# thanhndv212/figaroh-plus

Measured on AMD Instinct MI355X. Metric: samples/sec regressor build + TSQR solve, UR10 6-DoF, higher is better.
Workload: dtype f64

## Files before the change

figaroh_plus_amd/_lib.py:

```python
from __future__ import annotations

import ctypes as C
import os

import numpy as np

_HERE = os.path.dirname(os.path.abspath(__file__))
LIB_PATH = os.environ.get("FIGH_LIB_PATH") or os.path.join(_HERE, "libfigh.so")

ABI_VERSION = 116

FIGH_OK = 0
ERR_INVALID, ERR_NO_DEVICE, ERR_ALLOC, ERR_UNSUPPORTED, ERR_COMM = -1, -2, -3, -4, -5

MODE_JOINT_TORQUE, MODE_EXT_WRENCH = 0, 1
FLAG_FRICTION, FLAG_ACT_INERTIA, FLAG_OFFSET, FLAG_TX40, FLAG_GENERIC, FLAG_BLOCKED_INPUTS = 1, 2, 4, 8, 256, 512
FLAG_COMPACT_BLOCKS = 2048
FLAG_FORCE_COMPACT = 8192
FLAG_LINK_COMPACT = 4096
FLAG_ZEROS_PRESENT = 1024

_c_double_p = C.POINTER(C.c_double)
_c_int32_p = C.POINTER(C.c_int32)

SIGNATURES = {
# ... 48 lines not shown
    "figh_regressor_link_layout": (C.c_int, [C.c_void_p, C.c_int, C.c_int, C.c_int, _c_int32_p, C.POINTER(C.c_int)]),
    "figh_tsqr_selected_blocks": (C.c_int, [C.c_void_p, C.c_int64, C.c_int64, C.c_void_p, C.c_int, C.c_double, C.c_int,
                                            C.c_int, C.c_int, C.c_void_p, C.c_void_p, C.c_void_p, C.c_void_p, C.c_void_p,
                                            C.c_void_p, C.c_double, C.c_void_p, C.c_void_p, C.c_void_p]),
    "figh_block_rows_residuals": (C.c_int, [C.c_void_p, C.c_int, _c_int32_p, C.c_int, C.c_void_p, C.c_void_p]),
    "figh_tsqr_selected": (C.c_int, [C.c_void_p, C.c_int64, C.c_int64, C.c_void_p, C.c_int, C.c_double, C.c_int, C.c_int,
                                     C.c_int, C.c_void_p, C.c_double, C.c_void_p, C.c_void_p]),
    "figh_regressor_tsqr_fused": (C.c_int, [C.c_void_p, C.c_int, C.c_int64, C.c_void_p, C.c_void_p, C.c_void_p, C.c_void_p,
                                            C.c_int64, C.c_void_p, C.c_void_p, C.c_int, C.c_void_p, C.c_double,
                                            C.c_void_p]),
    "figh_chain_host_tail": (C.c_int, [C.c_void_p]),
    "figh_chain_pass_fused": (C.c_int, [C.c_void_p, C.c_int, C.c_int64, C.c_void_p, C.c_void_p, C.c_void_p, C.c_void_p,
                                        C.c_int64, C.c_void_p, C.c_int, C.c_void_p, C.c_double, C.c_double, C.c_void_p,
                                        C.c_void_p, C.c_size_t, C.c_void_p, C.POINTER(C.c_int), C.c_void_p]),
    "figh_tsqr_merge_base": (C.c_int, [C.c_void_p, C.c_int, C.c_int, C.c_int, C.c_double, C.c_void_p]),
    "figh_compact_rows": (C.c_int, [C.c_void_p, C.c_int64, C.c_int, C.c_int64, C.c_void_p, C.c_int, C.c_double, C.c_void_p,
                                    C.c_int64, C.c_void_p, C.POINTER(C.c_int64)]),
    "figh_base_permutation": (C.c_int, [C.c_void_p, C.c_int, C.c_int, C.c_double, C.c_void_p]),
    "figh_regressor_colsq": (C.c_int, [C.c_void_p, C.c_int, C.c_int, C.c_int, C.c_int64, C.c_void_p, C.c_void_p,
                                       C.c_void_p, C.c_int64, C.c_void_p]),
    "figh_regressor_tsqr": (C.c_int, [C.c_void_p, C.c_int, C.c_int, C.c_int, C.c_int64, C.c_void_p, C.c_void_p,
                                      C.c_void_p, C.c_void_p, C.c_int, C.c_void_p, _c_double_p, C.c_int, C.c_int64,
                                      C.c_void_p]),
    "figh_regressor_tsqr_norms": (C.c_int, [C.c_void_p, C.c_int, C.c_int, C.c_int, C.c_int64, C.c_void_p, C.c_void_p,
                                            C.c_void_p, C.c_void_p, C.c_int, C.c_void_p, _c_double_p, C.c_int, C.c_int64,
                                            C.c_void_p, C.c_void_p]),
    "figh_regressor_tsqr_batch": (C.c_int, [C.c_void_p, C.c_int, C.c_int, C.c_int, C.c_int64, C.c_int64, C.c_void_p,
                                            C.c_void_p, C.c_void_p, C.c_void_p, C.c_int, C.c_void_p, C.c_void_p]),
    "figh_regressor_tsqr_batch_fused": (C.c_int, [C.c_void_p, C.c_int, C.c_int64, C.c_int64, C.c_void_p, C.c_void_p,
                                                  C.c_void_p, C.c_void_p, C.c_int, C.c_void_p, C.c_void_p]),
# ... 652 lines not shown
                     kept_mask_u8, tail):
    changed = C.c_int(0)
    rc = load().figh_chain_pass_fused(model.handle, flags, N, d_q.ptr, d_v.ptr, d_a.ptr, d_W.ptr, ldw, d_kept.ptr, n,
                                      d_tau.ptr if d_tau is not None else None, tol_qr, tol_e, d_pack.ptr, h_pack, pack_bytes,
                                      kept_mask_u8.ctypes.data, C.byref(changed), tail.ref)
    if rc == ERR_UNSUPPORTED:
        return None
    check(rc)
    return not changed.value


def tsqr_merge_base(d_Rs, count, nc, n_free, tol_qr, d_Rk):
    check(load().figh_tsqr_merge_base(d_Rs.ptr, count, nc, n_free, tol_qr, d_Rk.ptr))


def repack_samples(d_src, N, width):
    d_dst = DeviceArray((((N + 63) // 64) * 64 * width,), np.float64)
    check(load().figh_repack_samples(d_src.ptr, N, width, d_dst.ptr))
    return d_dst
```

figaroh_plus_amd/csrc/figh_fused.hip:

```cpp
#include <algorithm>
#include <cmath>
#include <cstdlib>
#include <string>
#include <type_traits>

#include "figh_internal.h"
#include "figh_spatial.h"
#include "figh_chain.h"
#include "figh_wave.h"
#include "figh_tsqr_narrow.h"

namespace figh {

typedef double f64x2 __attribute__((ext_vector_type(2)));

struct FusedCtrl {
    int produced;
    int taken;
    int claimed;
    int pad[5];
};

__device__ __forceinline__ int lds_peek(const int *p) {
    return __hip_atomic_load(p, __ATOMIC_RELAXED, __HIP_MEMORY_SCOPE_WORKGROUP);
// ... 415 lines not shown
    if (!attr_set) {
        FIGH_HIP(hipFuncSetAttribute(reinterpret_cast<const void *>(&fused_chain_tsqr_kernel<NJ, TRAJ>),
                                     hipFuncAttributeMaxDynamicSharedMemorySize, 160 * 1024));
        attr_set = true;
    }
    plan->P = chain_params<NJ>(m);
    plan->tri = (int)tri;
    plan->ncons = ncons;
    plan->lds = sizeof(double) * (fixed + (size_t)ncons * tri);
    return FIGH_OK;
}

template <int NJ>
static int launch_fused(const figh_model_s *m, int flags, long N, const double *q, const double *v, const double *a,
                        double *W, const double *tau, const int *d_kept, int n, double *d_colsq, double **Rws_out,
                        long *count_out) {
    using G = FusedGeom<NJ>;
    const int nc = n + (tau ? 1 : 0);
    FusedPlan<NJ> pl;
    if (int rc = fused_plan<NJ, false>(m, nc, &pl)) return rc;
    const int cus = cu_count(), ncons = pl.ncons;
    const long ntiles_s = (N + 63) / 64;
    long grid = cus < ntiles_s / 2 ? cus : ntiles_s / 2;
    double *part = static_cast<double *>(workspace(sizeof(double) * grid * G::NPROD * G::NC, kWsRegressorNorms));
    double *Rws = static_cast<double *>(workspace(sizeof(double) * (size_t)nc * nc * (grid * ncons + 1), kWsLevel0TriOrWrench));
    if (!part || !Rws) return FIGH_ERR_ALLOC;
    {
        ProfileScope scope("fused_chain_tsqr", true);
        FIGH_LAUNCH_TIMED((fused_chain_tsqr_kernel<NJ, false>), dim3((unsigned)grid), dim3(64 * (G::NPROD + ncons)), pl.lds,
                          pl.P, flags, N, q, v, a, W, tau, d_kept, n, nc, part, Rws, ncons, pl.tri, null_pivot_sq());
    }
    launch_reduce_partials(part, (int)(grid * G::NPROD), G::NC, d_colsq);
    FIGH_HIP(hipGetLastError());
    *Rws_out = Rws;
    *count_out = grid * ncons;
    return FIGH_OK;
}

static long fused_batch_slices(long B, long n_per, int cus) {
    const long tiles = (n_per + 63) / 64;
    return std::max(1L, std::min(tiles, (long)cus / B));
}

template <int NJ>
static int launch_fused_batch(const figh_model_s *m, int flags, long B, long n_per, const double *q, const double *v,
                              const double *a, const int *d_cols, int n, const double *d_R_stack, double *d_R_out) {
    using G = FusedGeom<NJ>;
// ... 26 lines not shown
        FIGH_HIP(hipGetLastError());
        if (nb == 1) return FIGH_OK;
        cur = dst;
        cnt = nb;
        extra = nullptr;
        slot = slot == kWsMergeA ? kWsMergeB : kWsMergeA;
    }
}

}

using namespace figh;

static int fused_pass_launch(figh_model_t model, int flags, int64_t N, const double *d_q, const double *d_v, const double *d_a,
                             double *d_W, int64_t ldw, double *d_colsq, const int32_t *d_kept, int n, const double *d_tau,
                             double **Rws, long *count) {
    FIGH_REQUIRE(N >= 0 && n >= 1, "bad shape");
    const DevModel &h = model->host;
    const int nc = n + (d_tau ? 1 : 0);
    const int ncols = 14 * h.nlinks;
    if (!model->is_chain || (flags & (FIGH_FLAG_TX40 | FIGH_FLAG_GENERIC | FIGH_FLAG_BLOCKED_INPUTS)) || ldw != ncols ||
        (reinterpret_cast<uintptr_t>(d_W) % 16) != 0 || nc > 64 || n > ncols || N < 4096) {
        set_error("fused regressor + TSQR: serial chain, joint-torque mode, packed 16-byte aligned W, at most 64 columns "
                  "(tau included) and at least 4096 samples");
        return FIGH_ERR_UNSUPPORTED;
    }
    if (int rc = ensure_device()) return rc;
    const int f = flags & 7;
    switch (h.nlinks) {
        case 5:
            return launch_fused<5>(model, f, (long)N, d_q, d_v, d_a, d_W, d_tau, d_kept, n, d_colsq, Rws, count);
        case 6:
            return launch_fused<6>(model, f, (long)N, d_q, d_v, d_a, d_W, d_tau, d_kept, n, d_colsq, Rws, count);
        case 7:
            return launch_fused<7>(model, f, (long)N, d_q, d_v, d_a, d_W, d_tau, d_kept, n, d_colsq, Rws, count);
        default:
            set_error("fused regressor + TSQR: serial chains of 5 to 7 joints (LDS: two tile buffers + three consumer triangles)");
            return FIGH_ERR_UNSUPPORTED;
    }
}

extern "C" int figh_regressor_tsqr_fused(figh_model_t model, int flags, int64_t N, const double *d_q, const double *d_v,
                                         const double *d_a, double *d_W, int64_t ldw, double *d_colsq,
                                         const int32_t *d_kept, int n, const double *d_tau, double tol_qr,
                                         double *d_R_out) {
    FIGH_REQUIRE(model && d_q && d_v && d_a && d_W && d_colsq && d_kept && d_R_out, "NULL pointer");
    double *Rws = nullptr;
    long count = 0;
    if (int rc = fused_pass_launch(model, flags, N, d_q, d_v, d_a, d_W, ldw, d_colsq, d_kept, n, d_tau, &Rws, &count))
        return rc;
    return tsqr_reduce_stack(Rws, count, n + (d_tau ? 1 : 0), n, tol_qr, d_R_out);
}

extern "C" int figh_chain_pass_fused(figh_model_t model, int flags, int64_t N, const double *d_q, const double *d_v,
                                     const double *d_a, double *d_W, int64_t ldw, const int32_t *d_kept, int n,
                                     const double *d_tau, double tol_qr, double tol_e, double *d_pack, double *h_pack,
                                     size_t pack_bytes, const uint8_t *h_kept_mask, int *changed, figh_host_tail_t *tail) {
    FIGH_REQUIRE(model && d_q && d_v && d_a && d_W && d_kept && d_pack && h_pack && h_kept_mask && changed && tail,
                 "NULL pointer");
    FIGH_REQUIRE(tol_qr >= 0.0, "figh_chain_pass_fused: the rank decision needs tol_qr >= 0");
    const int ncols = 14 * model->host.nlinks, nc = n + (d_tau ? 1 : 0);
    const size_t sel_words = (size_t)(2 + 2 * ncols + 1) / 2;
    const size_t words = (size_t)ncols + sel_words + (size_t)(nc > 0 ? (nc + 1) * nc : 0);
    FIGH_REQUIRE(n >= 1 && pack_bytes >= sizeof(double) * words, "figh_chain_pass_fused: the pack is [colsq | sel | rows]");
    FIGH_REQUIRE(tail->n == n && (tail->with_tau != 0) == (d_tau != nullptr), "figh_chain_pass_fused: tail of another shape");
    double *d_colsq = d_pack, *d_rows = d_pack + ncols + sel_words;
    int32_t *d_sel = reinterpret_cast<int32_t *>(d_pack + ncols);
    double *Rws = nullptr;
    long count = 0;
    if (int rc = fused_pass_launch(model, flags, N, d_q, d_v, d_a, d_W, ldw, d_colsq, d_kept, n, d_tau, &Rws, &count)) return rc;
    if (int rc = tsqr_reduce_stack(Rws, count, nc, n, tol_qr, d_rows)) return rc;
    if (int rc = figh_select_columns(d_colsq, ncols, tol_e, 14, d_sel)) return rc;
    FIGH_HIP(hipMemcpyAsync(h_pack, d_pack, sizeof(double) * words, hipMemcpyDeviceToHost, stream()));
    FIGH_HIP(hipStreamSynchronize(stream()));
    const int32_t *mask_now = reinterpret_cast<const int32_t *>(h_pack + ncols) + 2 + ncols;
    *changed = 0;
    for (int c = 0; c < ncols; ++c)
        if ((mask_now[c] != 0) != (h_kept_mask[c] != 0)) {
            *changed = 1;
            return FIGH_OK;
        }
    tail->rows_k = h_pack + ncols + sel_words;
    return figh_chain_host_tail(tail);
}

static constexpr int64_t kFusedBatchMinSamples = 64;

extern "C" int figh_regressor_tsqr_batch_fused(figh_model_t model, int flags, int64_t B, int64_t n_per, const double *d_q,
// ... 40 lines not shown
```

figaroh_plus_amd/csrc/figh_internal.h:

```cpp
#pragma once

#include <hip/hip_runtime.h>
#include <hip/hip_ext.h>

#include <cstdint>
#include <cstdio>
#include <string>

#include "figh.h"

namespace figh {

constexpr int kMaxJoints = 64;

struct DevModel {
    int njoints, nq, nv, nlinks;
    int parents[kMaxJoints];
    int jtype[kMaxJoints];
    int idx_q[kMaxJoints];
    int idx_v[kMaxJoints];
    int body_mask[kMaxJoints];
    int depth[kMaxJoints];
    double axis[kMaxJoints][3];
    double placement[kMaxJoints][12];
// ... 172 lines not shown
    int njobs = 0, ncfull = 0, nfull = 0;
};
int launch_tsqr_group(std::vector<Tsqr2Job> &jobs, int ncfull, int nfull, int cus, GroupEmbed *later = nullptr);
int launch_tsqr_group_embed(const GroupEmbed &e);
int tsqr_reduce_stack(const double *d_Rs, long count, int nc, int n_free, double tol_qr, double *d_out);
int launch_tsqr_wide_pairs(const double *stack, long count, int nc, double *Rws_out);
int launch_tsqr_wide_single(const double *W, long rows, long ldw, const int *col_idx, int n, int nc, double *R_out);
int launch_tsqr_wide_batch(const double *W, long ldw, const int *col_idx, int n, int nc, long B, long n_per, int rps,
                           long seg_stride, long wgs, double *Rws_out);
int tsqr_wide_tile_rows(int nc);
int launch_tsqr_wide_chain(const double *W, long rows, long ldw, const int *col_idx, int n, const double *tau,
                           const double *d_blkw, long rows_per_blk, int nc, long nwg, double *Rws_out);

int launch_tsqr_tree(const double *Rs, long count, int nc, int n_free, double tol, double *d_out, double *d_rows_out);

int launch_tsqr_stream(const double *Rs, long count, int nc, int n_free, double tol, double *d_out, double *d_rows_out);

#define FIGH_HIP(expr)                                                                          \
    do {                                                                                        \
        hipError_t _e = (expr);                                                                 \
        if (_e != hipSuccess) {                                                                 \
            figh::set_error(std::string(#expr) + ": " + hipGetErrorString(_e));                 \
            return FIGH_ERR_NO_DEVICE;                                                          \
        }                                                                                       \
    } while (0)

#define FIGH_REQUIRE(cond, msg)              \
    do {                                     \
        if (!(cond)) {                       \
            figh::set_error(msg);            \
            return FIGH_ERR_INVALID;         \
// ... 5 lines not shown
```

figaroh_plus_amd/csrc/figh_linalg.hip:

```cpp
#include <cstdlib>
#include <algorithm>
#include <cstdio>
#include <type_traits>
#include <vector>

#include "figh_internal.h"
#include "figh_wave.h"
#include "figh_tsqr_narrow.h"
#include "figh_tsqr_narrow_kernel.h"

namespace figh {


template <int NCC, int NRC, bool LDSRED, bool RLAST = false>
__global__ __launch_bounds__(64, (NCC <= 4 || RLAST) ? 2 : 1) void tsqr2_kernel(
    const double *__restrict__ W, const long rows, const long ldw, const int *__restrict__ col_idx, const int n,
    const double *__restrict__ tau, const double *__restrict__ blkw, const long rows_per_blk,
    double *__restrict__ Rws, const int nc, const int *__restrict__ tile_first, const double null2) {
    tsqr2_level0_body<NCC, NRC, LDSRED, RLAST>(W, rows, ldw, col_idx, n, tau, blkw, rows_per_blk, Rws, nc, tile_first,
                                        (long)blockIdx.x, (long)gridDim.x, null2);
}



// ... 16 lines not shown
            s0 += x0 * x0;
            s1 += x1 * x1;
        }
        if (r < re) {
            const double x0 = W[r * ldw + c];
            s0 += x0 * x0;
        }
        part[(long)blockIdx.x * cols + c] = s0 + s1;
    }
}

__global__ __launch_bounds__(256) void reduce_partials_kernel(const double *__restrict__ part, int nblocks, int ncols,
                                                              double *__restrict__ out) {
    __shared__ double sm[256];
    const int c = blockIdx.x;
    double s = 0.0;
    for (int b = threadIdx.x; b < nblocks; b += 256) s += part[(long)b * ncols + c];
    sm[threadIdx.x] = s;
    __syncthreads();
    for (int w = 128; w > 0; w >>= 1) {
        if ((int)threadIdx.x < w) sm[threadIdx.x] += sm[threadIdx.x + w];
        __syncthreads();
    }
    if (threadIdx.x == 0) out[c] = sm[0];
}

void launch_reduce_partials(const double *part, int nblocks, int ncols, double *out) {
    hipLaunchKernelGGL(reduce_partials_kernel, dim3(ncols), dim3(256), 0, stream(), part, nblocks, ncols, out);
}

__global__ __launch_bounds__(256) void gather_cols_kernel(const double *__restrict__ W, long rows, long ldw,
                                                          const int *__restrict__ col_idx, int n,
                                                          double *__restrict__ out, long ldo) {
    const long total = rows * n;
    for (long e = (long)blockIdx.x * blockDim.x + threadIdx.x; e < total; e += (long)gridDim.x * blockDim.x) {
        const long r = e / n;
        const int c = (int)(e - r * n);
        out[r * ldo + c] = W[r * ldw + col_idx[c]];
// ... 83 lines not shown
            const int lim = 14 * b < ncols ? 14 * b : ncols;
            int f = 0;
            for (int c = 0; c < lim; ++c) f += kept[c];
            first[b] = f;
        }
        __syncthreads();
        const long t = (long)blockIdx.x * 256 + tid;
        if (t < ntiles) {
            const long r0 = t * 64, r1 = (r0 + 63 < rows ? r0 + 63 : rows - 1);
            int f = first[r0 / rows_per_block];
            for (long b = r0 / rows_per_block + 1; b <= r1 / rows_per_block; ++b) f = min(f, first[b]);
            tile_first[t] = f;
        }
    }
    if (blockIdx.x != 0) return;
    int total = 0;
    for (int c = 0; c < ncols; ++c) total += kept[c];
    for (int c = tid; c < ncols; c += 256) {
        int pos = 0;
        for (int e = 0; e < c; ++e) pos += kept[e];
        if (kept[c]) sel[2 + pos] = (link_pos ? max(link_pos[c / 14], 0) : c / 14) * link_stride + c % 14;
        if (c >= total) sel[2 + c] = 0;
        sel[2 + ncols + c] = kept[c];
    }
    if (tid == 0) {
        sel[0] = total;
        sel[1] = ncols;
    }
}

__global__ __launch_bounds__(256) void split_force_columns_kernel(const int *__restrict__ kept, const int n,
                                                                  const int link_stride, int *__restrict__ fsel,
                                                                  const int force_compact) {
    __shared__ int flag[1024];
    const int tid = threadIdx.x;
    for (int c = tid; c < n; c += 256) flag[c] = (kept[c] % link_stride) >= 6;
    __syncthreads();
    for (int c = tid; c < n; c += 256) {
        if (!flag[c]) continue;
        int pos = 0;
        for (int e = 0; e < c; ++e) pos += flag[e];
        const int p = kept[c] / link_stride, s = kept[c] % link_stride;
        fsel[pos] = force_compact ? 16 * (p >> 2) + 4 * (p & 3) + (s - 6) : kept[c];
// ... 496 lines not shown
int figh::tsqr_reduce_stack(const double *d_Rs, long count, int nc, int n_free, double tol_qr, double *d_out) {
    if (tol_qr < 0.0) return figh_tsqr_merge(d_Rs, (int)count, nc, d_out);
    double *one = static_cast<double *>(workspace(sizeof(double) * (size_t)nc * nc, kWsOneTri));
    if (!one) return FIGH_ERR_ALLOC;
    if (count == 1) {
        if (nc <= 80) return reveal_triangle(d_Rs, nc, n_free, tol_qr, d_out);
        FIGH_HIP(hipMemcpyAsync(one, d_Rs, sizeof(double) * (size_t)nc * nc, hipMemcpyDeviceToDevice, stream()));
        return reveal_triangle(one, nc, n_free, tol_qr, d_out);
    }
    if (nc <= 80) {
        const int rc = merge_one_launch(d_Rs, count, nc, n_free, tol_qr, one, d_out);
        if (rc != FIGH_ERR_UNSUPPORTED) return rc;
    }
    if (int rc = tsqr_reduce(d_Rs, count, nc, one)) return rc;
    return reveal_triangle(one, nc, n_free, tol_qr, d_out);
}

static int tsqr_selected_impl(const double *d_W, int64_t rows, int64_t ldw, const double *d_colsq, int ncols, double tol_e,
                              int link_stride, int nblocks, int n_expected, const double *d_tau, double tol_qr, int32_t *d_sel,
                              double *d_R_out, const int32_t *d_link_pos) {
    FIGH_REQUIRE(d_W && d_colsq && d_sel, "NULL device pointer");
    if (int rc = check_selected(ncols, link_stride, rows > 0 && n_expected <= ncols,
                                nblocks >= 0 && nblocks <= kMaxJoints && (nblocks == 0 || rows % nblocks == 0),
                                "rows must be a multiple of the hint blocks"))
        return rc;
    const int nc = n_expected + (d_tau ? 1 : 0);
    const bool hinted = nblocks > 0 && n_expected > 0 && nc <= 80 && rows / nblocks >= 1;
    const long ntiles = (rows + 63) / 64;
    int *d_tile = nullptr;
    if (hinted) {
// ... 299 lines not shown
    if (int rc = ensure_device()) return rc;
    ProfileScope scope("block_rows_residuals");
    hipLaunchKernelGGL(block_rows_residuals_kernel, dim3((unsigned)nblocks), dim3(256), 0, stream(), d_rows, bo, nc, d_v, d_r2);
    FIGH_HIP(hipGetLastError());
    return FIGH_OK;
}

int figh_tsqr_merge_base(const double *d_Rs, int count, int nc, int n_free, double tol_qr, double *d_Rk_out) {
    FIGH_REQUIRE(d_Rs && d_Rk_out, "NULL device pointer");
    FIGH_REQUIRE(count >= 1 && nc >= 1 && nc <= 512 && n_free >= 1 && n_free <= nc, "bad shape");
    FIGH_REQUIRE(tol_qr >= 0.0, "tol_qr must be non-negative");
    if (int rc = ensure_device()) return rc;
    return tsqr_reduce_stack(d_Rs, count, nc, n_free, tol_qr, d_Rk_out);
}

}
```

figaroh_plus_amd/csrc/figh_tsqr_stream.hip:

```cpp
#include "figh_internal.h"
#include "figh_wave.h"

namespace figh {

constexpr unsigned long long kPoison = 0xFFFBADC0FFEE5EEDull;
constexpr int kDepth = 1;

struct StreamPlan {
    int nlevels;
    int nb[6];
    int first[6];
    int nin[6];
};

__device__ __forceinline__ double ld_coherent(const double *p) {
    return __longlong_as_double(__hip_atomic_load(reinterpret_cast<const long long *>(p), __ATOMIC_RELAXED,
                                                  __HIP_MEMORY_SCOPE_AGENT));
}
__device__ __forceinline__ void st_coherent(double *p, const double v) {
    __hip_atomic_store(reinterpret_cast<long long *>(p), __double_as_longlong(v), __ATOMIC_RELAXED,
                       __HIP_MEMORY_SCOPE_AGENT);
}
__device__ __forceinline__ bool is_poison(const double v) { return (unsigned long long)__double_as_longlong(v) == kPoison; }

// ... 245 lines not shown
        if (c.lane_g == 0 && 16 * (P + cc) + c.lane_c >= c.pad) Rrow[16 * (P + cc) + c.lane_c] = 0.0 - wj;
    }
}

template <int P, int NCC>
__device__ __forceinline__ void solo_stream_panels(double (&T)[solo_tile_n(NCC)], double (&S)[kDepth][NCC], const SoloCtx &c) {
#define FIGH_RSTEP(KK) \
    if (16 * P + KK >= c.pad) solo_stream_step<KK, P, NCC>(T, S, c);
    FIGH_RSTEP(0) FIGH_RSTEP(1) FIGH_RSTEP(2) FIGH_RSTEP(3) FIGH_RSTEP(4) FIGH_RSTEP(5) FIGH_RSTEP(6) FIGH_RSTEP(7)
    FIGH_RSTEP(8) FIGH_RSTEP(9) FIGH_RSTEP(10) FIGH_RSTEP(11) FIGH_RSTEP(12) FIGH_RSTEP(13) FIGH_RSTEP(14)
    FIGH_RSTEP(15)
#undef FIGH_RSTEP
    if constexpr (P + 1 < NCC) solo_stream_panels<P + 1, NCC>(T, S, c);
}

template <int NCC, int FANR, int NW>
__global__ __launch_bounds__(64 * NW) void tsqr_stream_kernel(const double *in, double *sbuf, double *out, double *rows_out,
                                                              const StreamPlan plan, const int nc, const int n_free,
                                                              const double tol) {
    static_assert(NW == 8, "positions are dealt to eight waves");
    constexpr int FAN = 4 * FANR;
    __shared__ double pw[2][NW][16 * NCC];
    const int lane = threadIdx.x & 63, wave = __builtin_amdgcn_readfirstlane(threadIdx.x >> 6);
    const int lane_c = lane & 15, lane_g = lane >> 4;
    const int pad = 16 * NCC - nc;
    const int b = blockIdx.x;
    const long tri = (long)nc * nc;
    if (b < plan.first[plan.nlevels]) {
        int l = 0;
        while (l + 1 < plan.nlevels && b >= plan.first[l + 1]) ++l;
        const int bl = b - plan.first[l];
        const bool root = l == plan.nlevels - 1;
        MergeCtx<NCC, FANR> c;
        c.nc = nc;
        c.pad = pad;
        c.wave = wave;
        c.lane_c = lane_c;
// ... 15 lines not shown
            c.coff[r] = (c.have[r] ? ch : 0) * (int)tri + lane_c - pad;
        }
        c.stream = (!root || rows_out) ? sbuf + (long)b * tri : nullptr;
        c.plain = (root && out) ? out : nullptr;
        if (c.plain) {
            for (int e = threadIdx.x; e < nc * nc; e += 64 * NW) c.plain[e] = 0.0;
        }
        double T[merge_tile_n(NCC, FANR)];
#pragma unroll
        for (int e = 0; e < merge_tile_n(NCC, FANR); ++e) T[e] = 0.0;
        __syncthreads();
        stream_panels<0, NCC, FANR, NW>(T, c, pw);
        return;
    }
    for (int e = threadIdx.x; e < nc * nc; e += 64 * NW) rows_out[e] = 0.0;
    __syncthreads();
    if (wave != 0) return;
    SoloCtx c;
    c.nc = nc;
    c.pad = pad;
    c.lane_c = lane_c;
    c.lane_g = lane_g;
    c.n_free = n_free;
    c.tol = tol;
    c.rows_out = rows_out;
    if (plan.nlevels == 0) {
        c.R = in;
        c.repoison = nullptr;
    } else {
        double *rb = sbuf + (long)(plan.first[plan.nlevels] - 1) * tri;
// ... 5 lines not shown
    for (int e = 0; e < solo_tile_n(NCC); ++e) T[e] = 0.0;
#pragma unroll
    for (int dd = 0; dd < kDepth; ++dd)
#pragma unroll
        for (int e = 0; e < NCC; ++e) S[dd][e] = 0.0;
    solo_stream_panels<0, NCC>(T, S, c);
}

__global__ __launch_bounds__(256) void poison_fill_kernel(double *p, const long n) {
    for (long e = (long)blockIdx.x * 256 + threadIdx.x; e < n; e += (long)gridDim.x * 256)
        p[e] = __longlong_as_double((long long)kPoison);
}

template <int NCC, int FANR>
static int launch_stream(const double *Rs, long count, int nc, int n_free, double tol, double *d_out, double *d_rows_out,
                         int cus) {
    constexpr int FAN = 4 * FANR;
    StreamPlan plan{};
    int l = 0, total = 0;
    long cnt = count;
    while (cnt > 0) {
        if (l >= 5) return FIGH_ERR_UNSUPPORTED;
        const long nb = (cnt + FAN - 1) / FAN;
        plan.nin[l] = (int)cnt;
        plan.nb[l] = (int)nb;
        plan.first[l] = total;
        total += (int)nb;
        ++l;
        if (nb == 1) break;
        cnt = nb;
    }
    plan.nlevels = l;
    plan.first[l] = total;
    const int grid = total + (d_rows_out ? 1 : 0);
    if (grid > cus || grid < 1 || count * nc * nc >= (1L << 31)) return FIGH_ERR_UNSUPPORTED;
    static double *sbuf = nullptr;
    static long sbuf_elems = 0;
    const long need = (long)(total > 0 ? total : 1) * nc * nc;
    if (need > sbuf_elems) {
        if (sbuf) {
            FIGH_HIP(hipStreamSynchronize(stream()));
            FIGH_HIP(hipFree(sbuf));
            sbuf = nullptr;
            sbuf_elems = 0;
        }
        const long want = need + need / 4 + 4096;
        FIGH_HIP(hipMalloc(&sbuf, sizeof(double) * want));
        sbuf_elems = want;
        hipLaunchKernelGGL(poison_fill_kernel, dim3(256), dim3(256), 0, stream(), sbuf, want);
        FIGH_HIP(hipGetLastError());
    }
    static int occ = -1;
    if (occ < 0) {
        int v = 0;
        if (hipOccupancyMaxActiveBlocksPerMultiprocessor(&v, tsqr_stream_kernel<NCC, FANR, 8>, 512, 0) != hipSuccess) v = 0;
        occ = v;
    }
    if (occ < 1) return FIGH_ERR_UNSUPPORTED;
    hipLaunchKernelGGL((tsqr_stream_kernel<NCC, FANR, 8>), dim3((unsigned)grid), dim3(512), 0, stream(), Rs, sbuf, d_out,
                       d_rows_out, plan, nc, n_free, tol);
    FIGH_HIP(hipGetLastError());
    return FIGH_OK;
}

int launch_tsqr_stream(const double *Rs, long count, int nc, int n_free, double tol, double *d_out, double *d_rows_out) {
    int dev = 0, cus = 256;
    (void)hipGetDevice(&dev);
    if (hipDeviceGetAttribute(&cus, hipDeviceAttributeMultiprocessorCount, dev) != hipSuccess || cus <= 0) cus = 256;
    ProfileScope scope("tsqr_tree");
    if (nc <= 64) return launch_stream<4, 4>(Rs, count, nc, n_free, tol, d_out, d_rows_out, cus);
    if (nc <= 80) return launch_stream<5, 2>(Rs, count, nc, n_free, tol, d_out, d_rows_out, cus);
    return FIGH_ERR_UNSUPPORTED;
}

}
```

figaroh_plus_amd/pipeline.py:

```python
import numpy as np

from . import _lib
from .device import GpuMatrix
from .tools import qrdecomposition as qrd
from .tools.regressor import build_regressor_device


class Exchange:

    world_size = 1
    rank = 0

    @property
    def collective(self):
        return self.world_size > 1

    def sum_columns(self, d_colsq, ncols):
        return d_colsq.to_host()

    def sum_columns_device(self, d_colsq, ncols):
        if self.world_size > 1:
            total = np.ascontiguousarray(self.sum_columns(d_colsq, ncols), dtype=np.float64)
            _lib.check(_lib.load().figh_memcpy_h2d(d_colsq.ptr, total.ctypes.data, total.nbytes))

# ... 520 lines not shown
        pin = self._landing()
        total_rows = W.rows * ex.world_size
        tail = self._tail_args(n, with_tau, total_rows)
        ok = _lib.chain_pass_fused(handle, flags, self.N, self.d_q, self.d_v, self.d_a, W.buf, W.ld, d_kept, n, self.d_tau,
                                   self.tol_qr, self.tol_e, self._d_pack, pin.array.ctypes.data, 8 * pin.size,
                                   mask.view(np.uint8), tail)
        if ok is None:
            self.fuse = False
            return None
        if not ok:
            self._fused_kept = None
            return None
        self.fused_passes += 1
        self._n_expected = n
        idx_e, params_r = self._kept_lists(mask)
        out = self._native_out(tail, n, params_r, idx_e, pin.array[:ncols].copy(), with_tau, total_rows, strings)
        with _single_threaded_blas(n):
            pass
        return out

    def _tail_args(self, n, with_tau, total_rows):
        tail = self._host_tail
        if tail is None or tail.n != n or tail.with_tau != bool(with_tau):
            tail = self._host_tail = _lib.HostTail(n, with_tau)
        s = tail.s
        s.tol_qr, s.total_rows, s.pieces = self.tol_qr, int(total_rows), self._level0_pieces(total_rows)
        s.null_rule = int(self.null_pivots)
        if self._cert_cache is None or tail.cache_of is not self._cert_cache:
            s.n_cached_base = -1
        return tail

    def _native_out(self, tail, n, params_r, idx_e, col_norm, with_tau, total_rows, strings):
        s = tail.s
        r = s.n_base
# ... 300 lines not shown
```

include/figh.h:

```cpp
#ifndef FIGH_H
#define FIGH_H

#include <stddef.h>
#include <stdint.h>

#ifdef __cplusplus
extern "C" {
#endif

typedef enum {
    FIGH_OK = 0,
    FIGH_ERR_INVALID = -1,
    FIGH_ERR_NO_DEVICE = -2,
    FIGH_ERR_ALLOC = -3,
    FIGH_ERR_UNSUPPORTED = -4,
    FIGH_ERR_COMM = -5
} figh_status;

enum { FIGH_JT_REVOLUTE = 0, FIGH_JT_PRISMATIC = 1, FIGH_JT_CONTINUOUS = 2, FIGH_JT_FREEFLYER = 3, FIGH_JT_UNIVERSE = -1 };
enum { FIGH_MODE_JOINT_TORQUE = 0, FIGH_MODE_EXT_WRENCH = 1 };
enum { FIGH_FLAG_FRICTION = 1, FIGH_FLAG_ACT_INERTIA = 2, FIGH_FLAG_OFFSET = 4, FIGH_FLAG_TX40 = 8, FIGH_FLAG_GENERIC = 256,
       FIGH_FLAG_BLOCKED_INPUTS = 512,
       FIGH_FLAG_ZEROS_PRESENT = 1024,
       FIGH_FLAG_COMPACT_BLOCKS = 2048,
       FIGH_FLAG_LINK_COMPACT = 4096,
       FIGH_FLAG_FORCE_COMPACT = 8192 };

typedef struct figh_model_s *figh_model_t;

#define FIGH_ABI_VERSION 116
int figh_version(void);
const char *figh_last_error(void);
int figh_device_count(int *count);
int figh_device_set(int device);
int figh_host_wait_mode(int blocking);
int figh_tsqr_null_pivot_tol(double tol);
int figh_device_pci_bus_id(int device, char *out, int out_len);
int figh_device_info(char *name, int name_len, int *cu_count, size_t *hbm_bytes);
int figh_malloc(void **d_ptr, size_t bytes);
int figh_free(void *d_ptr);
int figh_memcpy_h2d(void *d_dst, const void *h_src, size_t bytes);
int figh_memcpy_d2h(void *h_dst, const void *d_src, size_t bytes);
int figh_host_alloc(void **h_ptr, size_t bytes);
int figh_host_free(void *h_ptr);
int figh_memcpy_d2d(void *d_dst, const void *d_src, size_t bytes);
// ... 71 lines not shown
int figh_chain_host_tail(figh_host_tail_t *tail);
int figh_chain_pass_fused(figh_model_t model, int flags, int64_t N, const double *d_q, const double *d_v, const double *d_a,
                          double *d_W, int64_t ldw, const int32_t *d_kept, int n, const double *d_tau, double tol_qr,
                          double tol_e, double *d_pack, double *h_pack, size_t pack_bytes, const uint8_t *h_kept_mask,
                          int *changed, figh_host_tail_t *tail);
int figh_tsqr_selected_wrench(const double *d_W, int64_t rows, int64_t ldw, const double *d_colsq, int ncols, double tol_e,
                              int link_stride, int n_expected, int nf_expected, const double *d_tau, double tol_qr,
                              int32_t *d_sel, double *d_R_out, const int32_t *d_link_pos, int64_t ld_force);
int figh_tsqr_selected_blocks(const double *d_W, int64_t rows, int64_t ldw, const double *d_colsq, int ncols, double tol_e,
                              int link_stride, int n_expected, int nblocks, const int32_t *h_counts, const int32_t *d_cols,
                              const int32_t *d_pos, const int64_t *h_block_off, const int32_t *h_block_ld,
                              const double *d_tau, double tol_qr, int32_t *d_sel, double *d_R_out, double *d_block_tri);
int figh_block_rows_residuals(const double *d_rows, int nblocks, const int32_t *h_row_off, int nc, const double *d_v,
                              double *d_r2);
int figh_tsqr_merge_base(const double *d_Rs, int count, int nc, int n_free, double tol_qr, double *d_rows_out);

int figh_regressor_colsq(figh_model_t model, int mode, int flags, int ft_mask, int64_t N, const double *d_q,
                         const double *d_v, const double *d_a, int64_t chunk_samples, double *d_colsq);
int figh_regressor_tsqr(figh_model_t model, int mode, int flags, int ft_mask, int64_t N, const double *d_q,
                        const double *d_v, const double *d_a, const int32_t *d_col_idx, int n, const double *d_tau,
                        const double *h_block_weight, int nblocks, int64_t chunk_samples, double *d_R_out);
int figh_regressor_tsqr_norms(figh_model_t model, int mode, int flags, int ft_mask, int64_t N, const double *d_q,
                              const double *d_v, const double *d_a, const int32_t *d_col_idx, int n, const double *d_tau,
                              const double *h_block_weight, int nblocks, int64_t chunk_samples, double *d_R_out,
                              double *d_colsq_out);
int figh_regressor_tsqr_batch(figh_model_t model, int mode, int flags, int ft_mask, int64_t B, int64_t n_per,
                              const double *d_q, const double *d_v, const double *d_a, const int32_t *d_col_idx, int n,
                              const double *d_R_stack, double *d_R_out);
int figh_regressor_tsqr_batch_fused(figh_model_t model, int flags, int64_t B, int64_t n_per, const double *d_q,
                                    const double *d_v, const double *d_a, const int32_t *d_col_idx, int n,
// ... 74 lines not shown
```

Baseline: 677.9 million.

## Fold partial reduction and column selection into the TSQR stream kernel, write to pinned host

```diff
diff --git a/figaroh_plus_amd/_lib.py b/figaroh_plus_amd/_lib.py
--- a/figaroh_plus_amd/_lib.py
+++ b/figaroh_plus_amd/_lib.py
@@ -8,7 +8,7 @@
 _HERE = os.path.dirname(os.path.abspath(__file__))
 LIB_PATH = os.environ.get("FIGH_LIB_PATH") or os.path.join(_HERE, "libfigh.so")
 
-ABI_VERSION = 116
+ABI_VERSION = 117
 
 FIGH_OK = 0
 ERR_INVALID, ERR_NO_DEVICE, ERR_ALLOC, ERR_UNSUPPORTED, ERR_COMM = -1, -2, -3, -4, -5
@@ -87,6 +87,8 @@
                                         C.c_int64, C.c_void_p, C.c_int, C.c_void_p, C.c_double, C.c_double, C.c_void_p,
                                         C.c_void_p, C.c_size_t, C.c_void_p, C.POINTER(C.c_int), C.c_void_p]),
     "figh_tsqr_merge_base": (C.c_int, [C.c_void_p, C.c_int, C.c_int, C.c_int, C.c_double, C.c_void_p]),
+    "figh_tsqr_merge_base_norms": (C.c_int, [C.c_void_p, C.c_int, C.c_int, C.c_int, C.c_double, C.c_void_p, C.c_int, C.c_int,
+                                             C.c_double, C.c_void_p, C.c_void_p, C.c_void_p]),
     "figh_compact_rows": (C.c_int, [C.c_void_p, C.c_int64, C.c_int, C.c_int64, C.c_void_p, C.c_int, C.c_double, C.c_void_p,
                                     C.c_int64, C.c_void_p, C.POINTER(C.c_int64)]),
     "figh_base_permutation": (C.c_int, [C.c_void_p, C.c_int, C.c_int, C.c_double, C.c_void_p]),
@@ -769,6 +771,11 @@
     check(load().figh_tsqr_merge_base(d_Rs.ptr, count, nc, n_free, tol_qr, d_Rk.ptr))
 
 
+def tsqr_merge_base_norms(d_Rs, count, nc, n_free, tol_qr, d_part, nblocks, ncols, tol_e, d_colsq, d_sel, d_Rk):
+    check(load().figh_tsqr_merge_base_norms(d_Rs.ptr, count, nc, n_free, tol_qr, d_part.ptr, nblocks, ncols, tol_e,
+                                            d_colsq.ptr, d_sel.ptr, d_Rk.ptr))
+
+
 def repack_samples(d_src, N, width):
     d_dst = DeviceArray((((N + 63) // 64) * 64 * width,), np.float64)
     check(load().figh_repack_samples(d_src.ptr, N, width, d_dst.ptr))
diff --git a/figaroh_plus_amd/csrc/figh_fused.hip b/figaroh_plus_amd/csrc/figh_fused.hip
--- a/figaroh_plus_amd/csrc/figh_fused.hip
+++ b/figaroh_plus_amd/csrc/figh_fused.hip
@@ -453,7 +453,7 @@
 template <int NJ>
 static int launch_fused(const figh_model_s *m, int flags, long N, const double *q, const double *v, const double *a,
                         double *W, const double *tau, const int *d_kept, int n, double *d_colsq, double **Rws_out,
-                        long *count_out) {
+                        long *count_out, const double **part_out, int *nparts_out) {
     using G = FusedGeom<NJ>;
     const int nc = n + (tau ? 1 : 0);
     FusedPlan<NJ> pl;
@@ -469,7 +469,12 @@
         FIGH_LAUNCH_TIMED((fused_chain_tsqr_kernel<NJ, false>), dim3((unsigned)grid), dim3(64 * (G::NPROD + ncons)), pl.lds,
                           pl.P, flags, N, q, v, a, W, tau, d_kept, n, nc, part, Rws, ncons, pl.tri, null_pivot_sq());
     }
-    launch_reduce_partials(part, (int)(grid * G::NPROD), G::NC, d_colsq);
+    if (part_out) {
+        *part_out = part;
+        *nparts_out = (int)(grid * G::NPROD);
+    } else {
+        launch_reduce_partials(part, (int)(grid * G::NPROD), G::NC, d_colsq);
+    }
     FIGH_HIP(hipGetLastError());
     *Rws_out = Rws;
     *count_out = grid * ncons;
@@ -526,7 +531,7 @@
 
 static int fused_pass_launch(figh_model_t model, int flags, int64_t N, const double *d_q, const double *d_v, const double *d_a,
                              double *d_W, int64_t ldw, double *d_colsq, const int32_t *d_kept, int n, const double *d_tau,
-                             double **Rws, long *count) {
+                             double **Rws, long *count, const double **part = nullptr, int *nparts = nullptr) {
     FIGH_REQUIRE(N >= 0 && n >= 1, "bad shape");
     const DevModel &h = model->host;
     const int nc = n + (d_tau ? 1 : 0);
@@ -541,11 +546,11 @@
     const int f = flags & 7;
     switch (h.nlinks) {
         case 5:
-            return launch_fused<5>(model, f, (long)N, d_q, d_v, d_a, d_W, d_tau, d_kept, n, d_colsq, Rws, count);
+            return launch_fused<5>(model, f, (long)N, d_q, d_v, d_a, d_W, d_tau, d_kept, n, d_colsq, Rws, count, part, nparts);
         case 6:
-            return launch_fused<6>(model, f, (long)N, d_q, d_v, d_a, d_W, d_tau, d_kept, n, d_colsq, Rws, count);
+            return launch_fused<6>(model, f, (long)N, d_q, d_v, d_a, d_W, d_tau, d_kept, n, d_colsq, Rws, count, part, nparts);
         case 7:
-            return launch_fused<7>(model, f, (long)N, d_q, d_v, d_a, d_W, d_tau, d_kept, n, d_colsq, Rws, count);
+            return launch_fused<7>(model, f, (long)N, d_q, d_v, d_a, d_W, d_tau, d_kept, n, d_colsq, Rws, count, part, nparts);
         default:
             set_error("fused regressor + TSQR: serial chains of 5 to 7 joints (LDS: two tile buffers + three consumer triangles)");
             return FIGH_ERR_UNSUPPORTED;
@@ -576,14 +581,37 @@
     const size_t words = (size_t)ncols + sel_words + (size_t)(nc > 0 ? (nc + 1) * nc : 0);
     FIGH_REQUIRE(n >= 1 && pack_bytes >= sizeof(double) * words, "figh_chain_pass_fused: the pack is [colsq | sel | rows]");
     FIGH_REQUIRE(tail->n == n && (tail->with_tau != 0) == (d_tau != nullptr), "figh_chain_pass_fused: tail of another shape");
-    double *d_colsq = d_pack, *d_rows = d_pack + ncols + sel_words;
-    int32_t *d_sel = reinterpret_cast<int32_t *>(d_pack + ncols);
+    double *pack = nullptr;
+    const bool on_host = hipHostGetDevicePointer(reinterpret_cast<void **>(&pack), h_pack, 0) == hipSuccess && pack;
+    if (!on_host) {
+        (void)hipGetLastError();
+        pack = d_pack;
+    }
     double *Rws = nullptr;
+    const double *part = nullptr;
     long count = 0;
-    if (int rc = fused_pass_launch(model, flags, N, d_q, d_v, d_a, d_W, ldw, d_colsq, d_kept, n, d_tau, &Rws, &count)) return rc;
-    if (int rc = tsqr_reduce_stack(Rws, count, nc, n, tol_qr, d_rows)) return rc;
-    if (int rc = figh_select_columns(d_colsq, ncols, tol_e, 14, d_sel)) return rc;
-    FIGH_HIP(hipMemcpyAsync(h_pack, d_pack, sizeof(double) * words, hipMemcpyDeviceToHost, stream()));
+    int nparts = 0;
+    if (int rc = fused_pass_launch(model, flags, N, d_q, d_v, d_a, d_W, ldw, d_pack, d_kept, n, d_tau, &Rws, &count, &part, &nparts))
+        return rc;
+    StreamEpilogue ep{};
+    ep.part = part;
+    ep.nblocks = nparts;
+    ep.ncols = ncols;
+    ep.tol_e = tol_e;
+    ep.link_stride = 14;
+    ep.colsq = pack;
+    ep.sel = reinterpret_cast<int32_t *>(pack + ncols);
+    ep.rows_on_host = on_host ? 1 : 0;
+    int rc = tsqr_reduce_stack_epilogue(Rws, count, nc, n, tol_qr, pack + ncols + sel_words, ep);
+    if (rc == FIGH_ERR_UNSUPPORTED && on_host) {
+        pack = d_pack;
+        ep.colsq = pack;
+        ep.sel = reinterpret_cast<int32_t *>(pack + ncols);
+        ep.rows_on_host = 0;
+        rc = tsqr_reduce_stack_epilogue(Rws, count, nc, n, tol_qr, pack + ncols + sel_words, ep);
+    }
+    if (rc) return rc;
+    if (pack == d_pack) FIGH_HIP(hipMemcpyAsync(h_pack, d_pack, sizeof(double) * words, hipMemcpyDeviceToHost, stream()));
     FIGH_HIP(hipStreamSynchronize(stream()));
     const int32_t *mask_now = reinterpret_cast<const int32_t *>(h_pack + ncols) + 2 + ncols;
     *changed = 0;
diff --git a/figaroh_plus_amd/csrc/figh_internal.h b/figaroh_plus_amd/csrc/figh_internal.h
--- a/figaroh_plus_amd/csrc/figh_internal.h
+++ b/figaroh_plus_amd/csrc/figh_internal.h
@@ -210,7 +210,20 @@
 
 int launch_tsqr_tree(const double *Rs, long count, int nc, int n_free, double tol, double *d_out, double *d_rows_out);
 
-int launch_tsqr_stream(const double *Rs, long count, int nc, int n_free, double tol, double *d_out, double *d_rows_out);
+constexpr int kEpilogueMaxCols = 128;
+struct StreamEpilogue {
+    const double *part;
+    int nblocks, ncols;
+    double tol_e;
+    int link_stride;
+    double *colsq;
+    int32_t *sel;
+    int rows_on_host;
+};
+int launch_tsqr_stream(const double *Rs, long count, int nc, int n_free, double tol, double *d_out, double *d_rows_out,
+                       const StreamEpilogue *ep = nullptr);
+int tsqr_reduce_stack_epilogue(const double *d_Rs, long count, int nc, int n_free, double tol_qr, double *d_out,
+                               const StreamEpilogue &ep);
 
 #define FIGH_HIP(expr)                                                                          \
     do {                                                                                        \
diff --git a/figaroh_plus_amd/csrc/figh_linalg.hip b/figaroh_plus_amd/csrc/figh_linalg.hip
--- a/figaroh_plus_amd/csrc/figh_linalg.hip
+++ b/figaroh_plus_amd/csrc/figh_linalg.hip
@@ -6,6 +6,7 @@
 
 #include "figh_internal.h"
 #include "figh_wave.h"
+#include "figh_pass_epilogue.h"
 #include "figh_tsqr_narrow.h"
 #include "figh_tsqr_narrow_kernel.h"
 
@@ -54,14 +55,7 @@
                                                               double *__restrict__ out) {
     __shared__ double sm[256];
     const int c = blockIdx.x;
-    double s = 0.0;
-    for (int b = threadIdx.x; b < nblocks; b += 256) s += part[(long)b * ncols + c];
-    sm[threadIdx.x] = s;
-    __syncthreads();
-    for (int w = 128; w > 0; w >>= 1) {
-        if ((int)threadIdx.x < w) sm[threadIdx.x] += sm[threadIdx.x + w];
-        __syncthreads();
-    }
+    reduce_partials_cols(part, nblocks, ncols, c, 1, sm, (int)threadIdx.x);
     if (threadIdx.x == 0) out[c] = sm[0];
 }
 
@@ -175,19 +169,7 @@
         }
     }
     if (blockIdx.x != 0) return;
-    int total = 0;
-    for (int c = 0; c < ncols; ++c) total += kept[c];
-    for (int c = tid; c < ncols; c += 256) {
-        int pos = 0;
-        for (int e = 0; e < c; ++e) pos += kept[e];
-        if (kept[c]) sel[2 + pos] = (link_pos ? max(link_pos[c / 14], 0) : c / 14) * link_stride + c % 14;
-        if (c >= total) sel[2 + c] = 0;
-        sel[2 + ncols + c] = kept[c];
-    }
-    if (tid == 0) {
-        sel[0] = total;
-        sel[1] = ncols;
-    }
+    select_columns_write(kept, ncols, link_stride, link_pos, sel, tid, 256);
 }
 
 __global__ __launch_bounds__(256) void split_force_columns_kernel(const int *__restrict__ kept, const int n,
@@ -714,6 +696,21 @@
     }
     if (int rc = tsqr_reduce(d_Rs, count, nc, one)) return rc;
     return reveal_triangle(one, nc, n_free, tol_qr, d_out);
+}
+
+int figh::tsqr_reduce_stack_epilogue(const double *d_Rs, long count, int nc, int n_free, double tol_qr, double *d_out,
+                                     const StreamEpilogue &ep) {
+    if (count > 1 && nc <= 80) {
+        double *one = static_cast<double *>(workspace(sizeof(double) * (size_t)nc * nc, kWsOneTri));
+        if (!one) return FIGH_ERR_ALLOC;
+        const int rc = launch_tsqr_stream(d_Rs, count, nc, n_free, tol_qr, one, d_out, &ep);
+        if (rc != FIGH_ERR_UNSUPPORTED) return rc;
+    }
+    if (ep.rows_on_host) return FIGH_ERR_UNSUPPORTED;
+    launch_reduce_partials(ep.part, ep.nblocks, ep.ncols, ep.colsq);
+    FIGH_HIP(hipGetLastError());
+    if (int rc = tsqr_reduce_stack(d_Rs, count, nc, n_free, tol_qr, d_out)) return rc;
+    return figh_select_columns(ep.colsq, ep.ncols, ep.tol_e, ep.link_stride, ep.sel);
 }
 
 static int tsqr_selected_impl(const double *d_W, int64_t rows, int64_t ldw, const double *d_colsq, int ncols, double tol_e,
@@ -1043,4 +1040,22 @@
     return tsqr_reduce_stack(d_Rs, count, nc, n_free, tol_qr, d_Rk_out);
 }
 
-}
+int figh_tsqr_merge_base_norms(const double *d_Rs, int count, int nc, int n_free, double tol_qr, const double *d_part,
+                               int nblocks, int ncols, double tol_e, double *d_colsq, int32_t *d_sel, double *d_rows_out) {
+    FIGH_REQUIRE(d_Rs && d_part && d_colsq && d_sel && d_rows_out, "NULL device pointer");
+    FIGH_REQUIRE(count >= 1 && nc >= 1 && nc <= 512 && n_free >= 1 && n_free <= nc, "bad shape");
+    FIGH_REQUIRE(nblocks >= 1 && ncols >= 1 && ncols <= 1024, "figh_tsqr_merge_base_norms: at least one block, 1 .. 1024 columns");
+    FIGH_REQUIRE(tol_qr >= 0.0, "tol_qr must be non-negative");
+    if (int rc = ensure_device()) return rc;
+    StreamEpilogue ep{};
+    ep.part = d_part;
+    ep.nblocks = nblocks;
+    ep.ncols = ncols;
+    ep.tol_e = tol_e;
+    ep.link_stride = 14;
+    ep.colsq = d_colsq;
+    ep.sel = d_sel;
+    return tsqr_reduce_stack_epilogue(d_Rs, count, nc, n_free, tol_qr, d_rows_out, ep);
+}
+
+}
diff --git a/figaroh_plus_amd/csrc/figh_pass_epilogue.h b/figaroh_plus_amd/csrc/figh_pass_epilogue.h
--- /dev/null
+++ b/figaroh_plus_amd/csrc/figh_pass_epilogue.h
@@ -0,0 +1,52 @@
+#pragma once
+
+#include "figh_internal.h"
+
+namespace figh {
+
+constexpr int kReduceCols = 8;
+
+static __device__ __noinline__ void reduce_partials_cols(const double *__restrict__ part, const int nblocks, const int ncols,
+                                                  const int c0, const int count, double *sm, const int t) {
+    double s[kReduceCols];
+#pragma unroll
+    for (int j = 0; j < kReduceCols; ++j) s[j] = 0.0;
+    for (int b = t; b < nblocks; b += 256) {
+        const double *row = part + (long)b * ncols + c0;
+#pragma unroll
+        for (int j = 0; j < kReduceCols; ++j)
+            if (j < count) s[j] += row[j];
+    }
+#pragma unroll
+    for (int j = 0; j < kReduceCols; ++j)
+        if (j < count) sm[256 * j + t] = s[j];
+    __syncthreads();
+    for (int w = 128; w > 0; w >>= 1) {
+        if (t < w) {
+#pragma unroll
+            for (int j = 0; j < kReduceCols; ++j)
+                if (j < count) sm[256 * j + t] += sm[256 * j + t + w];
+        }
+        __syncthreads();
+    }
+}
+
+static __device__ __noinline__ void select_columns_write(const int *kept, const int ncols, const int link_stride,
+                                                  const int *__restrict__ link_pos, int *__restrict__ sel, const int tid,
+                                                  const int nthreads) {
+    int total = 0;
+    for (int c = 0; c < ncols; ++c) total += kept[c];
+    for (int c = tid; c < ncols; c += nthreads) {
+        int pos = 0;
+        for (int e = 0; e < c; ++e) pos += kept[e];
+        if (kept[c]) sel[2 + pos] = (link_pos ? max(link_pos[c / 14], 0) : c / 14) * link_stride + c % 14;
+        if (c >= total) sel[2 + c] = 0;
+        sel[2 + ncols + c] = kept[c];
+    }
+    if (tid == 0) {
+        sel[0] = total;
+        sel[1] = ncols;
+    }
+}
+
+}
diff --git a/figaroh_plus_amd/csrc/figh_tsqr_stream.hip b/figaroh_plus_amd/csrc/figh_tsqr_stream.hip
--- a/figaroh_plus_amd/csrc/figh_tsqr_stream.hip
+++ b/figaroh_plus_amd/csrc/figh_tsqr_stream.hip
@@ -1,5 +1,6 @@
 #include "figh_internal.h"
 #include "figh_wave.h"
+#include "figh_pass_epilogue.h"
 
 namespace figh {
 
@@ -283,13 +284,37 @@
     if constexpr (P + 1 < NCC) solo_stream_panels<P + 1, NCC>(T, S, c);
 }
 
+__device__ __noinline__ void pass_epilogue(const StreamEpilogue ep, double *sm, int *kept, const int tid, const int nthreads) {
+    const int g = tid >> 8, t = tid & 255, ngroups = nthreads >> 8;
+    double *mine = sm + 256 * kReduceCols * g;
+    for (int r0 = 0; r0 < ep.ncols; r0 += kReduceCols * ngroups) {
+        const int c0 = r0 + kReduceCols * g;
+        const int left = ep.ncols - c0;
+        const int count = left < 0 ? 0 : (left < kReduceCols ? left : kReduceCols);
+        reduce_partials_cols(ep.part, ep.nblocks, ep.ncols, c0 < ep.ncols ? c0 : 0, count, mine, t);
+        if (t < count) {
+            const double v = mine[256 * t];
+            ep.colsq[c0 + t] = v;
+            kept[c0 + t] = !(v < ep.tol_e);
+        }
+        __syncthreads();
+    }
+    select_columns_write(kept, ep.ncols, ep.link_stride, nullptr, ep.sel, tid, nthreads);
+}
+
 template <int NCC, int FANR, int NW>
 __global__ __launch_bounds__(64 * NW) void tsqr_stream_kernel(const double *in, double *sbuf, double *out, double *rows_out,
                                                               const StreamPlan plan, const int nc, const int n_free,
-                                                              const double tol) {
+                                                              const double tol, const StreamEpilogue ep) {
     static_assert(NW == 8, "positions are dealt to eight waves");
     constexpr int FAN = 4 * FANR;
     __shared__ double pw[2][NW][16 * NCC];
+    if ((int)blockIdx.x > plan.first[plan.nlevels]) {
+        __shared__ double esm[(64 * NW / 256) * kReduceCols * 256];
+        __shared__ int ekept[kEpilogueMaxCols];
+        pass_epilogue(ep, esm, ekept, (int)threadIdx.x, 64 * NW);
+        return;
+    }
     const int lane = threadIdx.x & 63, wave = __builtin_amdgcn_readfirstlane(threadIdx.x >> 6);
     const int lane_c = lane & 15, lane_g = lane >> 4;
     const int pad = 16 * NCC - nc;
@@ -335,6 +360,7 @@
         return;
     }
     for (int e = threadIdx.x; e < nc * nc; e += 64 * NW) rows_out[e] = 0.0;
+    if (ep.rows_on_host) __threadfence_system();
     __syncthreads();
     if (wave != 0) return;
     SoloCtx c;
@@ -370,7 +396,7 @@
 
 template <int NCC, int FANR>
 static int launch_stream(const double *Rs, long count, int nc, int n_free, double tol, double *d_out, double *d_rows_out,
-                         int cus) {
+                         int cus, const StreamEpilogue *ep) {
     constexpr int FAN = 4 * FANR;
     StreamPlan plan{};
     int l = 0, total = 0;
@@ -388,7 +414,9 @@
     }
     plan.nlevels = l;
     plan.first[l] = total;
-    const int grid = total + (d_rows_out ? 1 : 0);
+    if (ep && (!ep->part || !d_rows_out || ep->ncols < 1 || ep->ncols > kEpilogueMaxCols || ep->nblocks < 0))
+        return FIGH_ERR_UNSUPPORTED;
+    const int grid = total + (d_rows_out ? 1 : 0) + (ep ? 1 : 0);
     if (grid > cus || grid < 1 || count * nc * nc >= (1L << 31)) return FIGH_ERR_UNSUPPORTED;
     static double *sbuf = nullptr;
     static long sbuf_elems = 0;
@@ -414,18 +442,19 @@
     }
     if (occ < 1) return FIGH_ERR_UNSUPPORTED;
     hipLaunchKernelGGL((tsqr_stream_kernel<NCC, FANR, 8>), dim3((unsigned)grid), dim3(512), 0, stream(), Rs, sbuf, d_out,
-                       d_rows_out, plan, nc, n_free, tol);
+                       d_rows_out, plan, nc, n_free, tol, ep ? *ep : StreamEpilogue{});
     FIGH_HIP(hipGetLastError());
     return FIGH_OK;
 }
 
-int launch_tsqr_stream(const double *Rs, long count, int nc, int n_free, double tol, double *d_out, double *d_rows_out) {
+int launch_tsqr_stream(const double *Rs, long count, int nc, int n_free, double tol, double *d_out, double *d_rows_out,
+                       const StreamEpilogue *ep) {
     int dev = 0, cus = 256;
     (void)hipGetDevice(&dev);
     if (hipDeviceGetAttribute(&cus, hipDeviceAttributeMultiprocessorCount, dev) != hipSuccess || cus <= 0) cus = 256;
     ProfileScope scope("tsqr_tree");
-    if (nc <= 64) return launch_stream<4, 4>(Rs, count, nc, n_free, tol, d_out, d_rows_out, cus);
-    if (nc <= 80) return launch_stream<5, 2>(Rs, count, nc, n_free, tol, d_out, d_rows_out, cus);
+    if (nc <= 64) return launch_stream<4, 4>(Rs, count, nc, n_free, tol, d_out, d_rows_out, cus, ep);
+    if (nc <= 80) return launch_stream<5, 2>(Rs, count, nc, n_free, tol, d_out, d_rows_out, cus, ep);
     return FIGH_ERR_UNSUPPORTED;
 }
 
diff --git a/figaroh_plus_amd/pipeline.py b/figaroh_plus_amd/pipeline.py
--- a/figaroh_plus_amd/pipeline.py
+++ b/figaroh_plus_amd/pipeline.py
@@ -558,10 +558,7 @@
         self.fused_passes += 1
         self._n_expected = n
         idx_e, params_r = self._kept_lists(mask)
-        out = self._native_out(tail, n, params_r, idx_e, pin.array[:ncols].copy(), with_tau, total_rows, strings)
-        with _single_threaded_blas(n):
-            pass
-        return out
+        return self._native_out(tail, n, params_r, idx_e, pin.array[:ncols].copy(), with_tau, total_rows, strings)
 
     def _tail_args(self, n, with_tau, total_rows):
         tail = self._host_tail
diff --git a/include/figh.h b/include/figh.h
--- a/include/figh.h
+++ b/include/figh.h
@@ -28,7 +28,7 @@
 
 typedef struct figh_model_s *figh_model_t;
 
-#define FIGH_ABI_VERSION 116
+#define FIGH_ABI_VERSION 117
 int figh_version(void);
 const char *figh_last_error(void);
 int figh_device_count(int *count);
@@ -130,6 +130,8 @@
 int figh_block_rows_residuals(const double *d_rows, int nblocks, const int32_t *h_row_off, int nc, const double *d_v,
                               double *d_r2);
 int figh_tsqr_merge_base(const double *d_Rs, int count, int nc, int n_free, double tol_qr, double *d_rows_out);
+int figh_tsqr_merge_base_norms(const double *d_Rs, int count, int nc, int n_free, double tol_qr, const double *d_part,
+                               int nblocks, int ncols, double tol_e, double *d_colsq, int32_t *d_sel, double *d_rows_out);
 
 int figh_regressor_colsq(figh_model_t model, int mode, int flags, int ft_mask, int64_t N, const double *d_q,
                          const double *d_v, const double *d_a, int64_t chunk_samples, double *d_colsq);
```

New measurement: 725.6 million (median of 6 runs). +7.0%, better.
